# lgautier/fastq-and-furious

Hardware: AMD Instinct MI355X
Metric: GB/s FASTQ parsed (higher is better)
Workload: dtype u8; 1 GPU; single-1g; description=S-single 150 bp synthetic FASTQ, 1073741522 bytes/GPU, 3334601 records/GPU, diagnostic=False, bytes_per_gpu=1073741522, records_per_gpu=3334601, total_bytes=1073741522, total_records=3334601

## Files before the change

### fastq-and-furious_amd/csrc/ffq_hip.hip

```cpp
#include "../../include/ffq.h"
#ifdef FFQ_PROBES
#include "../../include/ffq_probe.h"
#endif
#include "ffq_kernels.h"
#include "ffq_fasta.h"
#include "ffq_pool.h"

#include <hip/hip_runtime.h>
#include <hip/hip_ext.h>
#include <sys/mman.h>
#include <sys/stat.h>
#include <unistd.h>
#include <algorithm>
#include <cctype>
#include <chrono>
#include <cstdarg>
#include <cstdio>
#include <cstring>
#include <cstdlib>
#include <new>
#include <string>
#include <vector>

using namespace ffq;
// ... 68 lines not shown
    bool dense4_remember = false;
    int fused_skip = 0;
    int fused_backoff = HOLD_OFF;
    bool fz_in_place = false;
};

struct ffq_ctx {
    ScanState pend;
    ffq_ctx *owner = nullptr;
    StreamTail tail;
    bool owns_streams = true;
    double watchdog_s = 0;
    int device = 0;
    hipStream_t stream = nullptr;
    hipEvent_t ev[7] = {nullptr, nullptr, nullptr, nullptr, nullptr, nullptr, nullptr};
    InputMemory mem;
    RankBufs rk = {};
    int64_t rk_cap_tiles = 0, rk_cap_c = 0;
    uint8_t *fz_qphase = nullptr;
    int64_t fz_tiles_cap = 0;
    uint32_t *fz_bad = nullptr;
    bool decode_timed = false;
    int64_t cap_tiles = 0;
    uint16_t *ent = nullptr;
    uint32_t *cnt = nullptr;
    unsigned long long *ovf = nullptr;
    uint16_t *pool = nullptr;
    unsigned long long pool_cap = 0;
    int64_t cap_groups = 0;
    ChainBufs cb = {};
    int64_t stage_cap = 0;
    int64_t dstage_chunks = 0;
    long long *sbbase = nullptr;
    TileQ *tileq = nullptr;
    unsigned int *sbq = nullptr;
    long long *sbqbase = nullptr;
    Fast4Hdr *hdr4 = nullptr;
    TermInfo4 *tinfo4 = nullptr;
    Ctl *ctl = nullptr;
    LineIndex *d_L = nullptr;
    LineIndex *h_L = nullptr;
    DevRes *dres = nullptr;
    int64_t *qdir = nullptr;
    int64_t qdir_cap = 0;
    int64_t *p4s = nullptr;
    int64_t p4s_cap = 0;
    uint32_t *qrel = nullptr;
    Ctl *h_ctl = nullptr;
    DevRes *h_res = nullptr;
    Ctl *hm_ctl = nullptr;
    DevRes *hm_res = nullptr;
    unsigned long long *h_seq = nullptr, *hm_seq = nullptr;
    unsigned long long seq = 0;
    unsigned long long pub_seq = 0;
    bool ctl_clean = false;
    bool ctl_was_clean = false;
    int64_t *d_word = nullptr;
    int64_t *h_word = nullptr;
    int64_t *d_cut = nullptr, *h_cut = nullptr;
    FaHdr *fa_hdr = nullptr;
    uint8_t *stage_d = nullptr;
    int64_t stage_d_cap = 0;
    uint8_t *stage_h = nullptr;
    int64_t stage_h_cap = 0;
    int64_t *tab_d = nullptr;
    int64_t tab_d_cap = 0;
// ... 72 lines not shown
    }
    for (int i = 0; i < 7 && e == hipSuccess; i++)
        e = (i == 2 || i == 3) ? hipEventCreate(&c->ev[i])
                               : hipEventCreateWithFlags(&c->ev[i], hipEventDisableSystemFence);
    if (e == hipSuccess) e = hipMalloc((void **)&c->ctl, sizeof(Ctl));
    if (e == hipSuccess) e = hipMalloc((void **)&c->dres, sizeof(DevRes));
    if (e == hipSuccess) e = hipMalloc((void **)&c->d_L, sizeof(LineIndex));
    if (e == hipSuccess) e = hipMalloc((void **)&c->d_word, 16);
    if (e == hipSuccess) e = hipHostMalloc((void **)&c->h_word, 16, hipHostMallocDefault);
    if (e == hipSuccess) e = hipMalloc((void **)&c->d_cut, 48);
    if (e == hipSuccess) e = hipMalloc((void **)&c->fa_hdr, sizeof(FaHdr));
    if (e == hipSuccess) e = hipHostMalloc((void **)&c->h_cut, 48, hipHostMallocDefault);
    if (e == hipSuccess) e = hipHostMalloc((void **)&c->h_L, sizeof(LineIndex), hipHostMallocDefault);
    if (e == hipSuccess) e = hipHostMalloc((void **)&c->h_ctl, sizeof(Ctl), hipHostMallocMapped);
    if (e == hipSuccess) e = hipHostMalloc((void **)&c->h_res, sizeof(DevRes), hipHostMallocMapped);
    if (e == hipSuccess) e = hipHostMalloc((void **)&c->h_seq, 64, hipHostMallocMapped);
    if (e == hipSuccess) { *c->h_seq = 0; e = hipHostGetDevicePointer((void **)&c->hm_seq, c->h_seq, 0); }
    if (e == hipSuccess) e = hipHostGetDevicePointer((void **)&c->hm_ctl, c->h_ctl, 0);
    if (e == hipSuccess) e = hipHostGetDevicePointer((void **)&c->hm_res, c->h_res, 0);
    if (e != hipSuccess) {
        ffq_ctx_destroy(c);
        return fail(FFQ_E_HIP, "context setup failed: %s", hipGetErrorString(e));
    }
    *out = c;
    return FFQ_OK;
}

static void free_chain(ffq_ctx *c)
{
    (void)hipFree(c->cb.y); (void)hipFree(c->cb.exit); (void)hipFree(c->cb.cnt); (void)hipFree(c->cb.flags);
    (void)hipFree(c->cb.lines); (void)hipFree(c->cb.qb); (void)hipFree(c->cb.term); (void)hipFree(c->cb.stage);
    (void)hipFree(c->cb.rloc); (void)hipFree(c->cb.qloc); (void)hipFree(c->cb.part); (void)hipFree(c->cb.mins);
    (void)hipFree(c->cb.force); (void)hipFree(c->cb.dlist); (void)hipFree(c->cb.ilist);
    (void)hipFree(c->sbbase); (void)hipFree(c->tinfo4);
    (void)hipFree(c->tileq); (void)hipFree(c->sbq); (void)hipFree(c->sbqbase);
    c->sbbase = nullptr; c->tinfo4 = nullptr;
    c->tileq = nullptr; c->sbq = nullptr; c->sbqbase = nullptr;
    {
        StageRec *ds = c->cb.dstage; const int32_t dc = c->cb.dchunks;
        c->cb = ChainBufs{};
        c->cb.dstage = ds; c->cb.dchunks = dc;
    }
    c->stage_cap = 0;
    c->cap_groups = 0;
}

extern "C" int ffq_ctx_create_shared(ffq_ctx *parent, ffq_ctx **out)
{
    if (!parent || !out) return fail(FFQ_E_ARG, "ffq_ctx_create_shared: NULL argument");
    return ctx_create_impl(parent->device, parent, out);
}

extern "C" void ffq_ctx_destroy(ffq_ctx *c)
{
    if (!c) return;
    (void)hipSetDevice(c->device);
    if (c->stream) (void)hipStreamSynchronize(c->stream);
    stream_cache_drop(c);
    for (auto &r : c->stage_ev) for (auto &e : r) if (e) (void)hipEventDestroy(e);
    for (auto &st : c->stage_cs) if (st) { (void)hipStreamSynchronize(st); (void)hipStreamDestroy(st); }
    delete c->helpers;
    (void)hipFree(c->ent); (void)hipFree(c->cnt); (void)hipFree(c->ovf); (void)hipFree(c->pool);
    (void)hipFree(c->rk.tbase); (void)hipFree(c->rk.cand); (void)hipFree(c->rk.rec); (void)hipFree(c->rk.succ);
    (void)hipFree(c->rk.S[0]); (void)hipFree(c->rk.S[1]); (void)hipFree(c->rk.C[0]); (void)hipFree(c->rk.C[1]);
    (void)hipFree(c->rk.D); (void)hipFree(c->rk.root);
    free_chain(c);
    (void)hipFree(c->cb.dstage);
    (void)hipFree(c->fz_qphase); (void)hipFree(c->fz_bad);
    (void)hipFree(c->ctl); (void)hipFree(c->dres); (void)hipFree(c->d_L); (void)hipFree(c->hdr4);
// ... 95 lines not shown
constexpr int NMAX_FAST = PER_FAST * 64, NMAX_DENSE = PER_DENSE * 64;
constexpr int WPB_LITE = 2;

static int reserve_tiles(ffq_ctx *c, int64_t ntiles)
{
    if (ntiles <= c->cap_tiles) return FFQ_OK;
    CTX_SYNC(c);
    (void)hipFree(c->ent); (void)hipFree(c->cnt); (void)hipFree(c->ovf);
    c->ent = nullptr; c->cnt = nullptr; c->ovf = nullptr;
    free_chain(c);
    c->cap_tiles = 0;
    const int64_t ng = groups_for(ntiles);
    const int64_t nblk = (ng + RES_BLOCK - 1) / RES_BLOCK;
    HIPCHK(hipMalloc((void **)&c->ent, (size_t)ntiles * SLOT * sizeof(uint16_t)));
    HIPCHK(hipMalloc((void **)&c->cnt, (size_t)ntiles * sizeof(uint32_t)));
    HIPCHK(hipMalloc((void **)&c->ovf, (size_t)ntiles * sizeof(unsigned long long)));
    HIPCHK(hipMalloc((void **)&c->cb.y, (size_t)ng * 8));
    HIPCHK(hipMalloc((void **)&c->cb.exit, (size_t)ng * 8));
    HIPCHK(hipMalloc((void **)&c->cb.cnt, (size_t)ng * 4));
    HIPCHK(hipMalloc((void **)&c->cb.flags, (size_t)(2 * ng + 8) * 4));
    HIPCHK(hipMalloc((void **)&c->cb.dlist, (size_t)ng * 4));
    HIPCHK(hipMalloc((void **)&c->cb.ilist, (size_t)ng * 4));
    HIPCHK(hipMalloc((void **)&c->cb.lines, (size_t)ng * 4));
    HIPCHK(hipMalloc((void **)&c->cb.qb, (size_t)ng * 8));
    HIPCHK(hipMalloc((void **)&c->cb.term, (size_t)ng * sizeof(GroupTerm)));
    HIPCHK(hipMalloc((void **)&c->cb.rloc, (size_t)ng * 8));
    HIPCHK(hipMalloc((void **)&c->cb.qloc, (size_t)ng * 8));
    HIPCHK(hipMalloc((void **)&c->cb.part, (size_t)nblk * 4 * 8));
    HIPCHK(hipMalloc((void **)&c->cb.mins, 16));
    HIPCHK(hipMalloc((void **)&c->cb.force, (size_t)ng * 8));
    {
        const int64_t nsb = (ntiles + SB_TILES - 1) / SB_TILES;
        HIPCHK(hipMalloc((void **)&c->sbbase, (size_t)nsb * sizeof(long long)));
        HIPCHK(hipMalloc((void **)&c->tinfo4, (size_t)ntiles * sizeof(TermInfo4)));
        HIPCHK(hipMalloc((void **)&c->tileq, (size_t)ntiles * sizeof(TileQ)));
        HIPCHK(hipMalloc((void **)&c->sbq, (size_t)nsb * sizeof(unsigned int)));
        HIPCHK(hipMalloc((void **)&c->sbqbase, (size_t)nsb * sizeof(long long)));
        if (!c->hdr4) HIPCHK(hipMalloc((void **)&c->hdr4, sizeof(Fast4Hdr)));
    }
    c->cap_tiles = ntiles;
    c->cap_groups = ng;
    return FFQ_OK;
}

static int reserve_dstage(ffq_ctx *c, int64_t chunks)
{
    if (chunks <= c->dstage_chunks) return FFQ_OK;
    CTX_SYNC(c);
    (void)hipFree(c->cb.dstage);
    c->cb.dstage = nullptr; c->dstage_chunks = 0; c->cb.dchunks = 0;
    hipError_t e = hipMalloc((void **)&c->cb.dstage, (size_t)chunks * DCHUNK * sizeof(StageRec));
    if (e != hipSuccess) return fail(FFQ_E_NOMEM, "hipMalloc(walked groups' stage, %lld chunks) failed: %s", (long long)chunks, hipGetErrorString(e));
    c->dstage_chunks = chunks;
    c->cb.dchunks = (int32_t)chunks;
    return FFQ_OK;
}

static int reserve_stage(ffq_ctx *c, int64_t ng, int nmax)
{
    const int64_t need = ng * nmax;
    if (need <= c->stage_cap) return FFQ_OK;
    CTX_SYNC(c);
    (void)hipFree(c->cb.stage);
    c->cb.stage = nullptr; c->stage_cap = 0;
    hipError_t e = hipMalloc((void **)&c->cb.stage, (size_t)need * sizeof(StageRec));
    if (e != hipSuccess) return fail(FFQ_E_NOMEM, "hipMalloc(stage) failed: %s", hipGetErrorString(e));
// ... 297 lines not shown
    int rc = reserve_stage(c, ngroups, nmax);
    if (rc) return rc;
    rc = reserve_dstage(c, 64);
    if (rc) return rc;
    ChainBufs cb = chain_bufs(c, ngroups, nmax);
    hipStream_t sA = c->stream;
    HIPCHK(hipMemsetAsync(cb.flags, 0, (2 * (size_t)ngroups + 3) * 4, sA));
    static const bool no_lite = getenv("FFQ_NO_LITE") != nullptr;
    bool lite = !dense_cfg && !no_lite;
    if (lite && c->mem.lite_skip > 0) { c->mem.lite_skip--; lite = false; }
    st.lite_ran = lite;
    if (lite) {
        const int gl = lite_first_end_group(a.n_bytes, L.ntiles, ngroups);
        hipLaunchKernelGGL(HIP_KERNEL_NAME(k_chain_lite<WPB_LITE>), dim3((ngroups + WPB_LITE - 1) / WPB_LITE), dim3(WPB_LITE * 64), 0, sA,
                           L, a.offset, cb, ngroups, gl);
    }
    if (lite)
        hipLaunchKernelGGL(HIP_KERNEL_NAME(k_chain_wave_list<PER_FAST, EMAX_FAST, WPB_FAST, false>),
                           dim3(std::min((ngroups + WPB_FAST - 1) / WPB_FAST, 4096)), dim3(WPB_FAST * 64), 0, sA, L,
                           (const LineIndex *)c->d_L, a.offset, a.eof, cb);
    else if (!dense_cfg)
        hipLaunchKernelGGL(HIP_KERNEL_NAME(k_chain_wave<PER_FAST, EMAX_FAST, WPB_FAST, false>),
                           dim3((ngroups + WPB_FAST - 1) / WPB_FAST), dim3(WPB_FAST * 64), 0, sA, L,
                           (const LineIndex *)c->d_L, a.offset, a.eof, cb, 0, ngroups, 0);
    else
        hipLaunchKernelGGL(HIP_KERNEL_NAME(k_chain_wave<PER_DENSE, EMAX_DENSE, WPB_DENSE, true>),
                           dim3((ngroups + WPB_DENSE - 1) / WPB_DENSE), dim3(WPB_DENSE * 64), 0, sA, L,
                           (const LineIndex *)c->d_L, a.offset, a.eof, cb, 0, ngroups, 0);
    hipLaunchKernelGGL(k_dense_walk, dim3((unsigned)std::min((ngroups + 3) / 4, 1024)), dim3(256), 0, sA, L, cb, a.offset, a.eof, 1,
                       dense_cfg ? 1 : 0, c->ctl, 1);
    return enqueue_resolve(c, st, cb, timed, lite);
}

static void enqueue_sbscan(ffq_ctx *c, const LineIndex &L, int64_t ntiles, int nsb, int64_t offset)
{
    const unsigned int *presum = nullptr;
    if (nsb > 2048) {
        hipLaunchKernelGGL(k_sum64, dim3((unsigned)((nsb + 3) / 4)), dim3(256), 0, c->stream, (const uint32_t *)c->cnt, 1,
                           (int64_t)ntiles, c->sbq, nsb);
        presum = c->sbq;
    }
    hipLaunchKernelGGL(k_sbscan, dim3(1), dim3(1024), 0, c->stream, L, nsb, c->sbbase, offset, c->hdr4, presum);
}

static int end_front(ffq_ctx *c, const ScanState &st)
{
    const ScanArgs &a = st.a;
    c->pub_seq = 0;
    if (!st.poll_seq) HIPCHK(hipEventRecord(c->ev[3], c->stream));
    HIPCHK(hipGetLastError());
    StreamTail &tl = c->owner->tail;
    tl.is_scan = true;
    tl.out_p[0] = a.d_table; tl.out_n[0] = (size_t)a.table_cap * 48;
    tl.out_p[1] = st.decode ? a.d_qual : nullptr; tl.out_n[1] = st.decode ? (size_t)a.qual_cap : 0;
    tl.out_p[2] = st.decode ? a.d_qoff : nullptr; tl.out_n[2] = st.decode ? ((size_t)a.table_cap + 1) * 8 : 0;
    return FFQ_OK;
}

static int enqueue_front(ffq_ctx *c, ScanState &st)
{
    const ScanArgs &a = st.a;
    const bool serial = st.serial, decode = st.decode;
    hipStream_t sA = c->stream;
    const int64_t ntiles = st.ntiles;
    const int nsb = (int)((ntiles + SB_TILES - 1) / SB_TILES);
    if (c->mem.ranked_skip > 0 && !serial && !st.index_done) { c->mem.ranked_skip--; st.go_ranked = true; }
    if (st.force_ranked && !serial) st.go_ranked = true;
    st.probe4 = false;
    if (c->mem.fast4_remember && !st.fast4_failed) {
        st.fast4_failed = true;
        if (c->mem.fast4_skip > 0) c->mem.fast4_skip--;
        else st.probe4 = !serial && !st.go_ranked && !st.index_done;
    }
    if (c->mem.dense_skip > 0 && !st.dense_cfg && !st.index_done) { c->mem.dense_skip--; st.dense_cfg = true; }
    const bool try_fast4 = !serial && !st.go_ranked && !st.dense_cfg && !st.fast4_failed && !st.force_general &&
                           getenv("FFQ_NO_FAST4") == nullptr;
    const LineIndex L = make_index(c, a, ntiles);
    c->decode_timed = false;
    st.poll_seq = (st.poll_result && !decode) ? ++c->seq : 0;
    c->pub_seq = st.poll_seq;
    c->ctl_was_clean = c->ctl_clean;
    if (!c->ctl_clean) HIPCHK(hipMemsetAsync(c->ctl, 0, sizeof(Ctl), sA));
    c->ctl_clean = false;

    st.fused = false;
    st.in_place = (c->mem.fz_in_place || st.seg_refused) && a.qual_cap >= ntiles * (int64_t)TILE;
    if (decode && st.single_pass && try_fast4 && !st.index_done && !st.no_fused && a.offset < 16 &&
        (st.in_place || (!st.seg_refused && a.qual_cap >= ntiles * (int64_t)SG_STRIDE)) && (reinterpret_cast<uintptr_t>(a.d_qual) & 15) == 0) {
        if (c->mem.fused_skip > 0) c->mem.fused_skip--;
        else st.fused = true;
    }
    if (st.fused) {
        int rc = enqueue_fused_index(c, a, ntiles, st.in_place);
        if (rc) return rc;
        enqueue_sbscan(c, L, ntiles, nsb, a.offset);
        auto rows4 = st.in_place ? k_rows4<2, false> : k_rows4<1, false>;
        hipLaunchKernelGGL(rows4, dim3((unsigned)((ntiles + 3) / 4)), dim3(256), 0, sA, L,
                           (const long long *)c->sbbase, a.eof, a.add, c->hdr4, c->tinfo4, a.d_table, a.table_cap,
                           (uint32_t *)nullptr, c->tileq, (int64_t *)nullptr, a.table_cap,
                           (int64_t)(st.in_place ? TILE : SG_STRIDE), (const uint8_t *)c->fz_qphase, a.d_qoff);
        hipLaunchKernelGGL(k_finalize4, dim3(1), dim3(64), 0, sA, L, c->hdr4, (const TermInfo4 *)c->tinfo4, a.eof,
                           a.offset, a.add, (const int64_t *)a.d_table, a.table_cap, c->dres, no_pub(c), (const uint32_t *)c->fz_bad);
        hipLaunchKernelGGL(k_qtotal4, dim3(1), dim3(1), 0, sA, c->dres, (const int64_t *)a.d_table, a.table_cap,
                           a.d_qoff, make_pub(c));
        c->ctl_clean = true;
        st.stage = 1;
        return end_front(c, st);
    }

    st.untimed = st.no_timing && st.poll_seq && !st.index_done;
    bool any_order = st.untimed && c->ctl_was_clean;
    {
        const StreamTail &tl = c->owner->tail;
        if (!tl.is_scan || tl.exposed) any_order = false;
        const uintptr_t b0 = reinterpret_cast<uintptr_t>(a.d_buf), b1 = b0 + (size_t)a.n_bytes;
        for (int i = 0; i < 3 && any_order; i++) {
            const uintptr_t o0 = reinterpret_cast<uintptr_t>(tl.out_p[i]), o1 = o0 + tl.out_n[i];
            if (tl.out_p[i] && o0 < b1 && b0 < o1) any_order = false;
        }
    }
    static const bool no_wide = getenv("FFQ_NO_WIDE") != nullptr;
    if (!st.index_done)
        st.wide = decode && st.single_pass && !try_fast4 && !no_wide &&
                  a.qual_cap >= ntiles * (int64_t)TILE && (reinterpret_cast<uintptr_t>(a.d_qual) & 15) == 0;
    if (!st.untimed) HIPCHK(hipEventRecord(c->ev[0], sA));
    if (!st.index_done)
        launch_scan_lines(c, sA, a.d_buf, a.n_bytes, ntiles, L, (uint32_t)'@', any_order && !st.wide,
                          st.wide ? a.d_qual : (int8_t *)nullptr, a.qual_add);
    if (!st.untimed) HIPCHK(hipEventRecord(c->ev[1], sA));

    if (try_fast4) {
        enqueue_sbscan(c, L, ntiles, nsb, a.offset);
        if (decode) HIPCHK(hipMemsetAsync(c->tileq, 0, (size_t)ntiles * sizeof(TileQ), sA));
        if (c->mem.dense4_remember) st.dense4 = true;
        auto rows4 = st.dense4 ? k_rows4<false, true> : k_rows4<false, false>;
        hipLaunchKernelGGL(rows4, dim3((unsigned)((ntiles + 3) / 4)), dim3(256), 0, sA, L,
                           (const long long *)c->sbbase, a.eof, a.add, c->hdr4, c->tinfo4, a.d_table, a.table_cap,
                           decode ? c->qrel : (uint32_t *)nullptr, c->tileq, decode ? c->p4s : (int64_t *)nullptr,
                           decode ? std::min<int64_t>(a.table_cap, c->p4s_cap) : (int64_t)0,
                           (int64_t)0, (const uint8_t *)nullptr, (int64_t *)nullptr);
        hipLaunchKernelGGL(k_finalize4, dim3(1), dim3(64), 0, sA, L, c->hdr4, (const TermInfo4 *)c->tinfo4, a.eof,
                           a.offset, a.add, (const int64_t *)a.d_table, a.table_cap, c->dres,
                           decode ? no_pub(c) : make_pub(c));
        if (decode) {
            hipLaunchKernelGGL(k_sum64, dim3((unsigned)((nsb + 3) / 4)), dim3(256), 0, sA,
                               reinterpret_cast<const uint32_t *>(c->tileq) + 3, 4, (int64_t)ntiles, c->sbq, nsb);
            hipLaunchKernelGGL(k_qscan4, dim3(1), dim3(1024), 0, sA, (const unsigned int *)c->sbq, nsb, c->sbqbase);
            hipLaunchKernelGGL(k_qfix4, dim3((unsigned)((ntiles + 7) / 8)), dim3(256), 0, sA, (int)ntiles,
                               (const Fast4Hdr *)c->hdr4, (const TileQ *)c->tileq, (const long long *)c->sbqbase,
                               (const uint32_t *)c->qrel, a.d_qoff, std::min<int64_t>(a.table_cap, c->p4s_cap), c->qdir,
                               c->qdir_cap);
            hipLaunchKernelGGL(k_qtotal4, dim3(1), dim3(1), 0, sA, c->dres, (const int64_t *)a.d_table, a.table_cap,
                               a.d_qoff, make_pub(c));
            enqueue_decode(c, a, sA, true);
        }
        c->ctl_clean = true;
        st.stage = 1;
    } else {
        if (st.probe4) {
            enqueue_sbscan(c, L, ntiles, nsb, a.offset);
            auto rows4 = c->mem.dense4_remember ? k_rows4<false, true> : k_rows4<false, false>;
            hipLaunchKernelGGL(rows4, dim3((unsigned)((ntiles + 3) / 4)), dim3(256), 0, sA, L,
                               (const long long *)c->sbbase, a.eof, a.add, c->hdr4, c->tinfo4, a.d_table, a.table_cap,
                               (uint32_t *)nullptr, c->tileq, (int64_t *)nullptr, (int64_t)0,
                               (int64_t)0, (const uint8_t *)nullptr, (int64_t *)nullptr);
            hipLaunchKernelGGL(k_finalize4, dim3(1), dim3(64), 0, sA, L, c->hdr4, (const TermInfo4 *)c->tinfo4, a.eof,
                               a.offset, a.add, (const int64_t *)a.d_table, a.table_cap, c->dres, no_pub(c));
        }
        if (!serial && !st.go_ranked) {
            int rc = enqueue_general(c, st, L, true);
            if (rc) return rc;
        } else {
            hipLaunchKernelGGL(k_publish, dim3(1), dim3(1), 0, sA, c->dres, make_pub(c), 1);
            c->ctl_clean = true;
        }
        st.stage = 2;
    }
    return end_front(c, st);
}

template <class T>
static int grow_dev(ffq_ctx *c, T **p, int64_t *cap, int64_t need);

static int launch_scan_i64v(ffq_ctx *c, hipStream_t st, long long *v, int64_t nv, int64_t n_rows, DevRes *res)
{
    if (nv <= 2 * 32768) {
        hipLaunchKernelGGL(k_scan_i64v, dim3(1), dim3(1024), 0, st, v, nv, n_rows, res);
        return FFQ_OK;
    }
    const int64_t nb = (nv + SCAN_BLK - 1) / SCAN_BLK;
    int rc = grow_dev(c, &c->scan_bs, &c->scan_bs_cap, nb);
    if (rc) return rc;
    hipLaunchKernelGGL(k_scan_blksum, dim3((unsigned)nb), dim3(256), 0, st, (const long long *)v, nv, c->scan_bs);
    hipLaunchKernelGGL(k_scan_i64v, dim3(1), dim3(1024), 0, st, c->scan_bs, nb, n_rows, res);
    hipLaunchKernelGGL(k_scan_blkapply, dim3((unsigned)nb), dim3(256), 0, st, v, nv, (const long long *)c->scan_bs);
    return FFQ_OK;
}

static int launch_scan_u32(ffq_ctx *c, hipStream_t st, const unsigned int *v, int64_t nv, long long *base, long long *total)
// ... 942 lines not shown
```

### fastq-and-furious_amd/csrc/ffq_rows4.h

```cpp
#pragma once
#include "ffq_chain.h"

namespace ffq {

constexpr int SB_TILES = 64;
constexpr int R4_LIST = SLOT + 8;

struct Fast4Hdr {
    long long j0;
    int32_t attempt;
    int32_t dense_seen;
    unsigned long long irr_min;
    unsigned long long term_min;
    long long n_lines;
};

struct TermInfo4 {
    int64_t pos[6];
    int32_t status;
    int32_t final_;
};

struct TileQ {
    long long kfirst;
    int32_t nrec;
    uint32_t qsum;
};

__device__ __forceinline__ long long tile_ordinal_base(const LineIndex &L, const long long *sbbase, int t, int lane)
{
    const int sb = t / SB_TILES, t0 = sb * SB_TILES;
    const uint32_t c = (t0 + lane < t) ? L.cnt[t0 + lane] : 0u;
    return sbbase[sb] + (long long)wave_sum_u32(c) + L.s;
}

__global__ __launch_bounds__(256) void k_sum64(const uint32_t *__restrict__ src, int stride, int64_t nsrc,
                                               unsigned int *__restrict__ dst, int ndst)
{
    const int b = blockIdx.x * 4 + __builtin_amdgcn_readfirstlane((int)(threadIdx.x >> 6)), lane = threadIdx.x & 63;
    if (b >= ndst) return;
    const int64_t i = (int64_t)b * 64 + lane;
    const uint32_t v = (i < nsrc) ? src[i * stride] : 0u;
    const uint32_t t = wave_sum_u32(v);
    if (lane == 0) dst[b] = t;
}

__global__ __launch_bounds__(1024) void k_sbscan(LineIndex L, int nsb, long long *__restrict__ sbbase, int64_t offset,
                                                 Fast4Hdr *hdr, const unsigned int *__restrict__ presum)
{
    __shared__ long long s_w[16];
    __shared__ uint32_t s_sum[16][64];
    const int tid = threadIdx.x, lane = tid & 63, wid = tid >> 6;
    if (wid == 15) {
        const int tq = (int)min((int64_t)max(L.ntiles - 1, 0), max((int64_t)0, (offset - L.s) >> TILE_SHIFT));
        uint32_t sink = (L.n > 0) ? (uint32_t)L.d[0] : 0u;
        if (L.ntiles > 0) sink += L.cnt[tq] + L.ent[(int64_t)tq * SLOT + lane * 4];
        if (tq + 1 < L.ntiles) sink += L.cnt[tq + 1] + L.ent[(int64_t)(tq + 1) * SLOT + (lane & 15) * 4];
        asm volatile("" ::"v"(sink));
    }
    long long carry = 0;
    if (presum) {
        for (int c0 = 0; c0 < nsb; c0 += 16 * 1024) {
            uint32_t pv[16];
#pragma unroll
            for (int k = 0; k < 16; k++) {
                const int b = c0 + k * 1024 + tid;
                pv[k] = (b < nsb) ? presum[b] : 0u;
            }
#pragma unroll
            for (int k = 0; k < 16; k++) {
                const int b = c0 + k * 1024 + tid;
                if (c0 + k * 1024 >= nsb) continue;
                const uint32_t v = pv[k];
                const uint32_t incl = wave_incl_scan(v);
                if (lane == 63) s_w[wid] = (long long)incl;
                __syncthreads();
                long long wpre = 0, tot = 0;
// ... 27 lines not shown
                for (int q = 0; q < 4; q++)
                    if (t + q < L.ntiles) a += L.cnt[t + q];
                part[j] = a;
            }
        }
#pragma unroll
        for (int j = 0; j < 16; j++) {
            uint32_t r = part[j];
            r += (uint32_t)__builtin_amdgcn_update_dpp(0, (int)r, 0x111, 0xf, 0xf, false);
            r += (uint32_t)__builtin_amdgcn_update_dpp(0, (int)r, 0x112, 0xf, 0xf, false);
            r += (uint32_t)__builtin_amdgcn_update_dpp(0, (int)r, 0x114, 0xf, 0xf, false);
            r += (uint32_t)__builtin_amdgcn_update_dpp(0, (int)r, 0x118, 0xf, 0xf, false);
            if ((lane & 15) == 15) s_sum[wid][4 * j + (lane >> 4)] = r;
        }
        __syncthreads();
        const uint32_t v = (b < nsb) ? s_sum[wid][lane] : 0u;
        const uint32_t incl = wave_incl_scan(v);
        if (lane == 63) s_w[wid] = (long long)incl;
        __syncthreads();
        long long wpre = 0, tot = 0;
#pragma unroll
        for (int q = 0; q < 16; q++) {
            const long long t = s_w[q];
            if (q < wid) wpre += t;
            tot += t;
        }
        if (b < nsb) sbbase[b] = carry + wpre + (long long)(incl - v);
        __syncthreads();
        carry += tot;
    }
    __syncthreads();
    if (tid == 0) {
        hdr->n_lines = carry;
        hdr->irr_min = ~0ull;
        hdr->term_min = ~0ull;
        hdr->attempt = 1;
        hdr->dense_seen = 0;
        hdr->j0 = -1;
        const GAcc a(L);
        H h = a.before();
        long long ord = -1;
        long long found = -1;
        int64_t P; int fl;
        int tskip = (int)min((int64_t)L.ntiles, max((int64_t)0, (offset - L.s) >> TILE_SHIFT));
        if (tskip > 0) {
            long long o = sbbase[tskip / SB_TILES] + L.s;
            for (int t = (tskip / SB_TILES) * SB_TILES; t < tskip; t++) o += L.cnt[t];
            h = H{tskip - 1, 0x7FFFFFF0};
            ord = o - 1;
        }
        bool gave_up = false;
        for (int steps = 0;; steps++) {
            if (steps > 4096) { gave_up = true; break; }
            bool ok;
            if (h.tile >= 0 && h.i == 0x7FFFFFF0) {
                int t = h.tile + 1;
                while (t < L.ntiles && L.cnt[t] == 0) t++;
                ok = t < L.ntiles;
                if (ok) { h.tile = t; h.i = 0; }
            } else ok = a.next(h);
            if (!ok) break;
            ord++;
            a.get(h, P, fl);
            if ((fl & FL_AT) && P >= offset) { found = ord; break; }
        }
        if (gave_up) hdr->attempt = 0;
        else {
            hdr->j0 = found;
            if (found >= 0) {
                H h2 = h;
                if (a.next(h2) && a.next(h2)) {
                    a.get(h2, P, fl);
                    if (!(fl & FL_PLUS)) hdr->attempt = 0;
                }
            }
        }
    }
}

constexpr uint8_t FZ_ALL = 0xFE;
template <int FUSED, bool DENSE>
__global__ __launch_bounds__(256, DENSE ? 4 : 8) void k_rows4(LineIndex L, const long long *__restrict__ sbbase, int eof,
                                               int64_t add, Fast4Hdr *hdr, TermInfo4 *__restrict__ tinfo,
                                               int64_t *__restrict__ table, int64_t table_cap,
                                               uint32_t *__restrict__ qrel, TileQ *__restrict__ tileq,
                                               int64_t *__restrict__ p4s, int64_t p4_cap,
                                               int64_t fz_stride, const uint8_t *__restrict__ fz_phase,
                                               int64_t *__restrict__ fz_qoff)
{
    __shared__ __attribute__((aligned(16))) uint16_t s_ent_all[4][R4_LIST];
    __shared__ uint32_t s_la_all[4][8];
    __shared__ __attribute__((aligned(16))) int32_t s_rows_all[4][64 * 6];
    const int wid = __builtin_amdgcn_readfirstlane((int)(threadIdx.x >> 6)), lane = threadIdx.x & 63;
    const int t = blockIdx.x * 4 + wid;
    if (t >= L.ntiles) return;
    const int attempt = hdr->attempt;
    const long long j0 = hdr->j0;
    const unsigned long long irr0 = hdr->irr_min;
    const unsigned long long term0 = hdr->term_min;
    uint16_t *s_ent = s_ent_all[wid];
    uint32_t *s_la = s_la_all[wid];
    int32_t *s_rows = s_rows_all[wid];
    const int64_t len = L.len();

    const int tn = min(t + 1, L.ntiles - 1);
    const int sb = t / SB_TILES, t0 = sb * SB_TILES;
    const uint16_t *src = L.ent + (int64_t)t * SLOT;
    const uint32_t c_raw = L.cnt[t];
    const uint2 v0 = *reinterpret_cast<const uint2 *>(src + 4 * lane);
    const uint32_t c1_raw = L.cnt[tn];
    const uint2 vla_raw = *reinterpret_cast<const uint2 *>(L.ent + (int64_t)tn * SLOT + 4 * (lane & 1));
    const uint32_t cb_raw = L.cnt[min(t0 + lane, L.ntiles - 1)];
    const long long sbb = sbbase[sb];
    constexpr bool fused = FUSED != 0, in_place = FUSED == 2;
    uint32_t fzph = 0;
    if (fused) fzph = fz_phase[t];
    asm volatile("" ::"v"(c_raw), "v"(v0.x), "v"(v0.y), "v"(c1_raw), "v"(vla_raw.x), "v"(vla_raw.y), "v"(cb_raw),
                 "v"(sbb), "s"(attempt), "s"(j0), "v"(fzph));
    const int c = (int)c_raw;
    const bool have_next = t + 1 < L.ntiles;
    const int c1 = have_next ? (int)c1_raw : 0;
    const uint2 vla = vla_raw;
    const long long ob = sbb + (long long)wave_sum_u32((t0 + lane < t) ? cb_raw : 0u) + L.s;
    if (!attempt) return;
    if (ob - j0 > 0 && ((unsigned long long)((ob - j0) >> 2) > irr0 || (unsigned long long)((ob - j0) >> 2) > (term0 >> 24))) return;
    if (c > SLOT && (!DENSE || fused)) {
        if (lane == 0 && (hdr->irr_min != 0ull || !hdr->dense_seen)) { atomicMin(&hdr->irr_min, 0ull); hdr->dense_seen = 1; }
        return;
    }
    if (fused) {
        const uint32_t want = (uint32_t)(((j0 + 3 - ob) % 4 + 4) % 4);
        const bool wrong = in_place ? (fzph != (uint32_t)FZ_ALL && fzph != want) : (c > 0 && fzph != want);
        if ((wrong || j0 != 0) && lane == 0 && hdr->irr_min != 0ull) atomicMin(&hdr->irr_min, 0ull);
    }
    const int pre = (t == 0 && L.s) ? 1 : 0;
    if (c + pre == 0 && t != 0) return;
    const int64_t tbase = ((int64_t)t << TILE_SHIFT) + L.s;
    const int64_t tb_add = tbase + add;
    const int32_t lim = (int32_t)min(len - tbase, (int64_t)0x7FFFFFF0);
    if (j0 < 0) {
        if (t == 0 && lane == 0) {
            TermInfo4 &ti = tinfo[0];
            for (int i = 0; i < 6; i++) ti.pos[i] = -1;
            ti.status = ST_HEAD_BEG; ti.final_ = 0;
            atomicMin(&hdr->term_min, 0ull);
        }
        return;
    }
    const int ntot = pre + c;
    const int nch = DENSE ? (ntot + SLOT - 1) / SLOT : 1;
    const uint16_t *dsrc = nullptr;
    if (DENSE && c > SLOT) {
        const unsigned long long at = L.ovf[t] & OVF_MASK;
        if (at + (unsigned long long)c > L.pool_cap) {
            if (lane == 0) atomicMin(&hdr->irr_min, 0ull);
            return;
// ... 336 lines not shown
        if (r + 1 >= me.nrec) nxt = me.qsum;
        else if (lane == 63) nxt = (idx + 1 < table_cap) ? (int64_t)qrel[idx + 1] : (int64_t)me.qsum;
        if (act) {
            qoff[idx] = base + loc;
            qdir_mark(qdir, qdir_cap, base + loc, nxt - loc, idx);
        }
    };
    auto rest = [&](const TileQ &me, int64_t base) {
        for (int r0 = 64; r0 < me.nrec; r0 += 64) {
            const int64_t idx = me.kfirst + r0 + lane;
            const bool act = r0 + lane < me.nrec && idx < table_cap;
            fix(me, base, r0, act ? (int64_t)qrel[idx] : 0, act);
        }
    };
    if (me0.nrec > 0) fix(me0, base0, 0, l0, a0);
    if (me1.nrec > 0) fix(me1, base1, 0, l1, a1);
    if (me0.nrec > 64) rest(me0, base0);
    if (me1.nrec > 64) rest(me1, base1);
}

__global__ void k_qtotal4(DevRes *res, const int64_t *__restrict__ table, int64_t table_cap,
                          int64_t *__restrict__ qoff, Pub pb)
{
    if (threadIdx.x != 0 || blockIdx.x != 0) return;
    if (res->fallback) { publish(pb, res); return; }
    const int64_t n = res->n_records;
    int64_t tot = 0;
    if (n > 0 && n <= table_cap) tot = qoff[n - 1] + (table[(n - 1) * 6 + 5] - table[(n - 1) * 6 + 4]);
    res->n_qual_bytes = tot;
    if (n <= table_cap) qoff[n] = tot;
    publish(pb, res);
}

__global__ void k_finalize4(LineIndex L, Fast4Hdr *hdr, const TermInfo4 *__restrict__ tinfo, int eof,
                            int64_t offset, int64_t add, const int64_t *__restrict__ table, int64_t table_cap,
                            DevRes *res, Pub pb, const uint32_t *__restrict__ fz_bad = nullptr)
{
    if (threadIdx.x != 0 || blockIdx.x != 0) return;
    res->n_lines = hdr->n_lines;
    res->n_qual_bytes = 0;
    res->term_group = -1;
    res->has_final = 0;
    const unsigned long long tm = hdr->term_min, im = hdr->irr_min;
    const unsigned long long tk = tm >> 24;
    res->fused_bad = fz_bad ? (int32_t)*fz_bad : 0;
    res->fast4_dense = hdr->dense_seen;
    if (!hdr->attempt || tm == ~0ull || (im != ~0ull && im <= tk) || (fz_bad && *fz_bad)) { res->fallback = 1; res->fast4_hint = 0; publish(pb, res); return; }
    res->fallback = 0;
    res->fast4_hint = 1;
    const int tt = (int)(tm & 0xFFFFFF);
    const TermInfo4 ti = tinfo[tt];
    const int status = ti.status;
    res->last_status = status;
    for (int i = 0; i < 6; i++) res->last_pos[i] = (ti.pos[i] >= 0) ? ti.pos[i] + add : -1;
    const long long ncomplete = (long long)tk;
    res->n_records = ncomplete + (ti.final_ ? 1 : 0);
    res->has_final = ti.final_ ? 1 : 0;
    int end;
    if (ti.final_) end = 0;
    else if (status == ST_HEAD_BEG) end = eof ? 0 : 1;
    else if (eof) end = (status == ST_QUAL_END) ? 2 : (status == ST_INVALID) ? 4 : 3;
    else end = (status == ST_INVALID) ? 4 : 1;
    res->end_state = end;
    if (ncomplete > 0 && ncomplete <= table_cap) res->end_offset = table[(ncomplete - 1) * 6 + 5] - add - 1;
    else res->end_offset = offset;
    publish(pb, res);
}

}
```

Measured before the change: 4976 GB/s.

## Replace single-block superblock scan with multi-block two-level ordinal base

```diff
diff --git a/fastq-and-furious_amd/csrc/ffq_hip.hip b/fastq-and-furious_amd/csrc/ffq_hip.hip
--- a/fastq-and-furious_amd/csrc/ffq_hip.hip
+++ b/fastq-and-furious_amd/csrc/ffq_hip.hip
@@ -124,6 +124,8 @@
     int64_t stage_cap = 0;
     int64_t dstage_chunks = 0;
     long long *sbbase = nullptr;
+    uint32_t *sbsum = nullptr;
+    uint32_t *blksum = nullptr;
     TileQ *tileq = nullptr;
     unsigned int *sbq = nullptr;
     long long *sbqbase = nullptr;
@@ -262,9 +264,9 @@
     (void)hipFree(c->cb.lines); (void)hipFree(c->cb.qb); (void)hipFree(c->cb.term); (void)hipFree(c->cb.stage);
     (void)hipFree(c->cb.rloc); (void)hipFree(c->cb.qloc); (void)hipFree(c->cb.part); (void)hipFree(c->cb.mins);
     (void)hipFree(c->cb.force); (void)hipFree(c->cb.dlist); (void)hipFree(c->cb.ilist);
-    (void)hipFree(c->sbbase); (void)hipFree(c->tinfo4);
+    (void)hipFree(c->sbbase); (void)hipFree(c->tinfo4); (void)hipFree(c->sbsum); (void)hipFree(c->blksum);
     (void)hipFree(c->tileq); (void)hipFree(c->sbq); (void)hipFree(c->sbqbase);
-    c->sbbase = nullptr; c->tinfo4 = nullptr;
+    c->sbbase = nullptr; c->tinfo4 = nullptr; c->sbsum = nullptr; c->blksum = nullptr;
     c->tileq = nullptr; c->sbq = nullptr; c->sbqbase = nullptr;
     {
         StageRec *ds = c->cb.dstage; const int32_t dc = c->cb.dchunks;
@@ -426,6 +428,8 @@
     {
         const int64_t nsb = (ntiles + SB_TILES - 1) / SB_TILES;
         HIPCHK(hipMalloc((void **)&c->sbbase, (size_t)nsb * sizeof(long long)));
+        HIPCHK(hipMalloc((void **)&c->sbsum, (size_t)nsb * sizeof(uint32_t)));
+        HIPCHK(hipMalloc((void **)&c->blksum, (size_t)OB_MAXBLK * sizeof(uint32_t)));
         HIPCHK(hipMalloc((void **)&c->tinfo4, (size_t)ntiles * sizeof(TermInfo4)));
         HIPCHK(hipMalloc((void **)&c->tileq, (size_t)ntiles * sizeof(TileQ)));
         HIPCHK(hipMalloc((void **)&c->sbq, (size_t)nsb * sizeof(unsigned int)));
@@ -789,8 +793,16 @@
     return enqueue_resolve(c, st, cb, timed, lite);
 }
 
-static void enqueue_sbscan(ffq_ctx *c, const LineIndex &L, int64_t ntiles, int nsb, int64_t offset)
-{
+static OrdBase enqueue_obase(ffq_ctx *c, const LineIndex &L, int64_t ntiles, int nsb, int64_t offset)
+{
+    OrdBase ob{c->sbbase, c->sbsum, c->blksum, 0};
+    const int64_t nblk = (ntiles + BLK_TILES - 1) / BLK_TILES;
+    if (nblk <= OB_MAXBLK && offset - L.s < TILE) {
+        hipLaunchKernelGGL(k_obase, dim3((unsigned)(nblk + 1)), dim3(64), 0, c->stream, L, (int)nblk, nsb, c->sbsum,
+                           c->blksum, offset, c->hdr4);
+        ob.nblk = (int32_t)nblk;
+        return ob;
+    }
     const unsigned int *presum = nullptr;
     if (nsb > 2048) {
         hipLaunchKernelGGL(k_sum64, dim3((unsigned)((nsb + 3) / 4)), dim3(256), 0, c->stream, (const uint32_t *)c->cnt, 1,
@@ -798,6 +810,7 @@
         presum = c->sbq;
     }
     hipLaunchKernelGGL(k_sbscan, dim3(1), dim3(1024), 0, c->stream, L, nsb, c->sbbase, offset, c->hdr4, presum);
+    return ob;
 }
 
 static int end_front(ffq_ctx *c, const ScanState &st)
@@ -850,13 +863,13 @@
     if (st.fused) {
         int rc = enqueue_fused_index(c, a, ntiles, st.in_place);
         if (rc) return rc;
-        enqueue_sbscan(c, L, ntiles, nsb, a.offset);
+        const OrdBase ob = enqueue_obase(c, L, ntiles, nsb, a.offset);
         auto rows4 = st.in_place ? k_rows4<2, false> : k_rows4<1, false>;
         hipLaunchKernelGGL(rows4, dim3((unsigned)((ntiles + 3) / 4)), dim3(256), 0, sA, L,
-                           (const long long *)c->sbbase, a.eof, a.add, c->hdr4, c->tinfo4, a.d_table, a.table_cap,
+                           ob, a.eof, a.add, c->hdr4, c->tinfo4, a.d_table, a.table_cap,
                            (uint32_t *)nullptr, c->tileq, (int64_t *)nullptr, a.table_cap,
                            (int64_t)(st.in_place ? TILE : SG_STRIDE), (const uint8_t *)c->fz_qphase, a.d_qoff);
-        hipLaunchKernelGGL(k_finalize4, dim3(1), dim3(64), 0, sA, L, c->hdr4, (const TermInfo4 *)c->tinfo4, a.eof,
+        hipLaunchKernelGGL(k_finalize4, dim3(1), dim3(64), 0, sA, L, c->hdr4, ob, (const TermInfo4 *)c->tinfo4, a.eof,
                            a.offset, a.add, (const int64_t *)a.d_table, a.table_cap, c->dres, no_pub(c), (const uint32_t *)c->fz_bad);
         hipLaunchKernelGGL(k_qtotal4, dim3(1), dim3(1), 0, sA, c->dres, (const int64_t *)a.d_table, a.table_cap,
                            a.d_qoff, make_pub(c));
@@ -887,16 +900,16 @@
     if (!st.untimed) HIPCHK(hipEventRecord(c->ev[1], sA));
 
     if (try_fast4) {
-        enqueue_sbscan(c, L, ntiles, nsb, a.offset);
+        const OrdBase ob = enqueue_obase(c, L, ntiles, nsb, a.offset);
         if (decode) HIPCHK(hipMemsetAsync(c->tileq, 0, (size_t)ntiles * sizeof(TileQ), sA));
         if (c->mem.dense4_remember) st.dense4 = true;
         auto rows4 = st.dense4 ? k_rows4<false, true> : k_rows4<false, false>;
         hipLaunchKernelGGL(rows4, dim3((unsigned)((ntiles + 3) / 4)), dim3(256), 0, sA, L,
-                           (const long long *)c->sbbase, a.eof, a.add, c->hdr4, c->tinfo4, a.d_table, a.table_cap,
+                           ob, a.eof, a.add, c->hdr4, c->tinfo4, a.d_table, a.table_cap,
                            decode ? c->qrel : (uint32_t *)nullptr, c->tileq, decode ? c->p4s : (int64_t *)nullptr,
                            decode ? std::min<int64_t>(a.table_cap, c->p4s_cap) : (int64_t)0,
                            (int64_t)0, (const uint8_t *)nullptr, (int64_t *)nullptr);
-        hipLaunchKernelGGL(k_finalize4, dim3(1), dim3(64), 0, sA, L, c->hdr4, (const TermInfo4 *)c->tinfo4, a.eof,
+        hipLaunchKernelGGL(k_finalize4, dim3(1), dim3(64), 0, sA, L, c->hdr4, ob, (const TermInfo4 *)c->tinfo4, a.eof,
                            a.offset, a.add, (const int64_t *)a.d_table, a.table_cap, c->dres,
                            decode ? no_pub(c) : make_pub(c));
         if (decode) {
@@ -915,13 +928,13 @@
         st.stage = 1;
     } else {
         if (st.probe4) {
-            enqueue_sbscan(c, L, ntiles, nsb, a.offset);
+            const OrdBase ob = enqueue_obase(c, L, ntiles, nsb, a.offset);
             auto rows4 = c->mem.dense4_remember ? k_rows4<false, true> : k_rows4<false, false>;
             hipLaunchKernelGGL(rows4, dim3((unsigned)((ntiles + 3) / 4)), dim3(256), 0, sA, L,
-                               (const long long *)c->sbbase, a.eof, a.add, c->hdr4, c->tinfo4, a.d_table, a.table_cap,
+                               ob, a.eof, a.add, c->hdr4, c->tinfo4, a.d_table, a.table_cap,
                                (uint32_t *)nullptr, c->tileq, (int64_t *)nullptr, (int64_t)0,
                                (int64_t)0, (const uint8_t *)nullptr, (int64_t *)nullptr);
-            hipLaunchKernelGGL(k_finalize4, dim3(1), dim3(64), 0, sA, L, c->hdr4, (const TermInfo4 *)c->tinfo4, a.eof,
+            hipLaunchKernelGGL(k_finalize4, dim3(1), dim3(64), 0, sA, L, c->hdr4, ob, (const TermInfo4 *)c->tinfo4, a.eof,
                                a.offset, a.add, (const int64_t *)a.d_table, a.table_cap, c->dres, no_pub(c));
         }
         if (!serial && !st.go_ranked) {
diff --git a/fastq-and-furious_amd/csrc/ffq_rows4.h b/fastq-and-furious_amd/csrc/ffq_rows4.h
--- a/fastq-and-furious_amd/csrc/ffq_rows4.h
+++ b/fastq-and-furious_amd/csrc/ffq_rows4.h
@@ -4,7 +4,16 @@
 namespace ffq {
 
 constexpr int SB_TILES = 64;
+constexpr int BLK_TILES = SB_TILES * 64;
+constexpr int OB_MAXBLK = 64;
 constexpr int R4_LIST = SLOT + 8;
+
+struct OrdBase {
+    const long long *sbbase;
+    const uint32_t *sbsum;
+    const uint32_t *blksum;
+    int32_t nblk;
+};
 
 struct Fast4Hdr {
     long long j0;
@@ -43,6 +52,53 @@
     const uint32_t v = (i < nsrc) ? src[i * stride] : 0u;
     const uint32_t t = wave_sum_u32(v);
     if (lane == 0) dst[b] = t;
+}
+
+__device__ void fast4_first(const LineIndex &L, const long long *sbbase, int64_t offset, Fast4Hdr *hdr)
+{
+    hdr->irr_min = ~0ull;
+    hdr->term_min = ~0ull;
+    hdr->attempt = 1;
+    hdr->dense_seen = 0;
+    hdr->j0 = -1;
+    const GAcc a(L);
+    H h = a.before();
+    long long ord = -1;
+    long long found = -1;
+    int64_t P; int fl;
+    int tskip = (int)min((int64_t)L.ntiles, max((int64_t)0, (offset - L.s) >> TILE_SHIFT));
+    if (tskip > 0) {
+        long long o = sbbase[tskip / SB_TILES] + L.s;
+        for (int t = (tskip / SB_TILES) * SB_TILES; t < tskip; t++) o += L.cnt[t];
+        h = H{tskip - 1, 0x7FFFFFF0};
+        ord = o - 1;
+    }
+    bool gave_up = false;
+    for (int steps = 0;; steps++) {
+        if (steps > 4096) { gave_up = true; break; }
+        bool ok;
+        if (h.tile >= 0 && h.i == 0x7FFFFFF0) {
+            int t = h.tile + 1;
+            while (t < L.ntiles && L.cnt[t] == 0) t++;
+            ok = t < L.ntiles;
+            if (ok) { h.tile = t; h.i = 0; }
+        } else ok = a.next(h);
+        if (!ok) break;
+        ord++;
+        a.get(h, P, fl);
+        if ((fl & FL_AT) && P >= offset) { found = ord; break; }
+    }
+    if (gave_up) hdr->attempt = 0;
+    else {
+        hdr->j0 = found;
+        if (found >= 0) {
+            H h2 = h;
+            if (a.next(h2) && a.next(h2)) {
+                a.get(h2, P, fl);
+                if (!(fl & FL_PLUS)) hdr->attempt = 0;
+            }
+        }
+    }
 }
 
 __global__ __launch_bounds__(1024) void k_sbscan(LineIndex L, int nsb, long long *__restrict__ sbbase, int64_t offset,
@@ -136,55 +192,86 @@
     __syncthreads();
     if (tid == 0) {
         hdr->n_lines = carry;
-        hdr->irr_min = ~0ull;
-        hdr->term_min = ~0ull;
-        hdr->attempt = 1;
-        hdr->dense_seen = 0;
-        hdr->j0 = -1;
-        const GAcc a(L);
-        H h = a.before();
-        long long ord = -1;
-        long long found = -1;
-        int64_t P; int fl;
-        int tskip = (int)min((int64_t)L.ntiles, max((int64_t)0, (offset - L.s) >> TILE_SHIFT));
-        if (tskip > 0) {
-            long long o = sbbase[tskip / SB_TILES] + L.s;
-            for (int t = (tskip / SB_TILES) * SB_TILES; t < tskip; t++) o += L.cnt[t];
-            h = H{tskip - 1, 0x7FFFFFF0};
-            ord = o - 1;
-        }
-        bool gave_up = false;
-        for (int steps = 0;; steps++) {
-            if (steps > 4096) { gave_up = true; break; }
-            bool ok;
-            if (h.tile >= 0 && h.i == 0x7FFFFFF0) {
-                int t = h.tile + 1;
-                while (t < L.ntiles && L.cnt[t] == 0) t++;
-                ok = t < L.ntiles;
-                if (ok) { h.tile = t; h.i = 0; }
-            } else ok = a.next(h);
-            if (!ok) break;
-            ord++;
-            a.get(h, P, fl);
-            if ((fl & FL_AT) && P >= offset) { found = ord; break; }
-        }
-        if (gave_up) hdr->attempt = 0;
-        else {
-            hdr->j0 = found;
-            if (found >= 0) {
-                H h2 = h;
-                if (a.next(h2) && a.next(h2)) {
-                    a.get(h2, P, fl);
-                    if (!(fl & FL_PLUS)) hdr->attempt = 0;
-                }
-            }
-        }
-    }
+        fast4_first(L, sbbase, offset, hdr);
+    }
+}
+
+__global__ __launch_bounds__(64) void k_obase(LineIndex L, int nblk, int nsb, uint32_t *__restrict__ sbsum,
+                                              uint32_t *__restrict__ blksum, int64_t offset, Fast4Hdr *hdr)
+{
+    const int lane = threadIdx.x;
+    if (blockIdx.x == 0) {
+        const bool have0 = L.ntiles > 0;
+        const uint32_t c0 = have0 ? L.cnt[0] : 0u;
+        const uint2 v = have0 ? *reinterpret_cast<const uint2 *>(L.ent + 4 * lane) : make_uint2(0u, 0u);
+        const uint8_t b0 = L.n > 0 ? L.d[0] : 0;
+        const int nin = (c0 <= (uint32_t)SLOT) ? min((int)c0, 256) : 0;
+        const uint32_t x[4] = {v.x & 0xFFFFu, v.x >> 16, v.y & 0xFFFFu, v.y >> 16};
+        int q0 = 4;
+#pragma unroll
+        for (int q = 3; q >= 0; q--)
+            if (4 * lane + q < nin && ((x[q] >> 14) & FL_AT) && (int64_t)(x[q] & OFF_MASK) + L.s >= offset) q0 = q;
+        const unsigned long long m = __ballot(q0 < 4);
+        long long j0 = -1;
+        int e2 = -1;
+        if (L.s && b0 == '@' && offset <= 0) { j0 = 0; e2 = 1; }
+        else if (m != 0ull) {
+            const int fl = __ffsll((long long)m) - 1;
+            const int i = 4 * fl + __shfl(q0, fl);
+            j0 = L.s + i; e2 = i + 2;
+        }
+        const bool decided = e2 >= 0 && e2 < nin;
+        const uint32_t w = (uint32_t)__shfl((int)((e2 & 2) ? v.y : v.x), (e2 >> 2) & 63);
+        const uint32_t fl2 = ((e2 & 1) ? (w >> 16) : (w & 0xFFFFu)) >> 14;
+        if (lane == 0) {
+            if (decided) {
+                hdr->irr_min = ~0ull;
+                hdr->term_min = ~0ull;
+                hdr->dense_seen = 0;
+                hdr->j0 = j0;
+                hdr->attempt = (fl2 & FL_PLUS) ? 1 : 0;
+            } else fast4_first(L, nullptr, offset, hdr);
+        }
+        return;
+    }
+    const int b = blockIdx.x - 1;
+    const int64_t tw0 = (int64_t)b * BLK_TILES + lane * 4;
+    uint32_t part[16];
+    if ((int64_t)(b + 1) * BLK_TILES <= L.ntiles) {
+        uint4 xx[16];
+#pragma unroll
+        for (int j = 0; j < 16; j++) xx[j] = *reinterpret_cast<const uint4 *>(L.cnt + tw0 + ((int64_t)j << 8));
+#pragma unroll
+        for (int j = 0; j < 16; j++) part[j] = xx[j].x + xx[j].y + xx[j].z + xx[j].w;
+    } else {
+#pragma unroll
+        for (int j = 0; j < 16; j++) {
+            const int64_t t = tw0 + ((int64_t)j << 8);
+            uint32_t a = 0;
+            for (int q = 0; q < 4; q++)
+                if (t + q < L.ntiles) a += L.cnt[t + q];
+            part[j] = a;
+        }
+    }
+    uint32_t tot = 0;
+#pragma unroll
+    for (int j = 0; j < 16; j++) {
+        uint32_t r = part[j];
+        tot += r;
+        r += (uint32_t)__builtin_amdgcn_update_dpp(0, (int)r, 0x111, 0xf, 0xf, false);
+        r += (uint32_t)__builtin_amdgcn_update_dpp(0, (int)r, 0x112, 0xf, 0xf, false);
+        r += (uint32_t)__builtin_amdgcn_update_dpp(0, (int)r, 0x114, 0xf, 0xf, false);
+        r += (uint32_t)__builtin_amdgcn_update_dpp(0, (int)r, 0x118, 0xf, 0xf, false);
+        const int s = b * 64 + 4 * j + (lane >> 4);
+        if ((lane & 15) == 15 && s < nsb) sbsum[s] = r;
+    }
+    tot = wave_sum_u32(tot);
+    if (lane == 0) blksum[b] = tot;
 }
 
 constexpr uint8_t FZ_ALL = 0xFE;
 template <int FUSED, bool DENSE>
-__global__ __launch_bounds__(256, DENSE ? 4 : 8) void k_rows4(LineIndex L, const long long *__restrict__ sbbase, int eof,
+__global__ __launch_bounds__(256, DENSE ? 4 : 8) void k_rows4(LineIndex L, const OrdBase obase, int eof,
                                                int64_t add, Fast4Hdr *hdr, TermInfo4 *__restrict__ tinfo,
                                                int64_t *__restrict__ table, int64_t table_cap,
                                                uint32_t *__restrict__ qrel, TileQ *__restrict__ tileq,
@@ -209,23 +296,30 @@
 
     const int tn = min(t + 1, L.ntiles - 1);
     const int sb = t / SB_TILES, t0 = sb * SB_TILES;
+    const int blk = t / BLK_TILES, s0 = blk * 64;
     const uint16_t *src = L.ent + (int64_t)t * SLOT;
     const uint32_t c_raw = L.cnt[t];
     const uint2 v0 = *reinterpret_cast<const uint2 *>(src + 4 * lane);
     const uint32_t c1_raw = L.cnt[tn];
     const uint2 vla_raw = *reinterpret_cast<const uint2 *>(L.ent + (int64_t)tn * SLOT + 4 * (lane & 1));
     const uint32_t cb_raw = L.cnt[min(t0 + lane, L.ntiles - 1)];
-    const long long sbb = sbbase[sb];
+    const uint32_t sbs_raw = obase.sbsum[min(s0 + lane, (L.ntiles - 1) / SB_TILES)];
+    const uint32_t bls_raw = obase.blksum[min(lane, OB_MAXBLK - 1)];
+    const long long sbb_raw = obase.sbbase[sb];
     constexpr bool fused = FUSED != 0, in_place = FUSED == 2;
     uint32_t fzph = 0;
     if (fused) fzph = fz_phase[t];
     asm volatile("" ::"v"(c_raw), "v"(v0.x), "v"(v0.y), "v"(c1_raw), "v"(vla_raw.x), "v"(vla_raw.y), "v"(cb_raw),
-                 "v"(sbb), "s"(attempt), "s"(j0), "v"(fzph));
+                 "v"(sbs_raw), "v"(bls_raw), "v"(sbb_raw), "s"(attempt), "s"(j0), "v"(fzph));
     const int c = (int)c_raw;
     const bool have_next = t + 1 < L.ntiles;
     const int c1 = have_next ? (int)c1_raw : 0;
     const uint2 vla = vla_raw;
-    const long long ob = sbb + (long long)wave_sum_u32((t0 + lane < t) ? cb_raw : 0u) + L.s;
+    const bool two = obase.nblk > 0;
+    const long long sbb = two ? 0ll : sbb_raw;
+    const uint32_t lsum = ((t0 + lane < t) ? cb_raw : 0u) + ((two && s0 + lane < sb) ? sbs_raw : 0u) +
+                          ((two && lane < blk) ? bls_raw : 0u);
+    const long long ob = sbb + (long long)wave_sum_u32(lsum) + L.s;
     if (!attempt) return;
     if (ob - j0 > 0 && ((unsigned long long)((ob - j0) >> 2) > irr0 || (unsigned long long)((ob - j0) >> 2) > (term0 >> 24))) return;
     if (c > SLOT && (!DENSE || fused)) {
@@ -628,12 +722,18 @@
     publish(pb, res);
 }
 
-__global__ void k_finalize4(LineIndex L, Fast4Hdr *hdr, const TermInfo4 *__restrict__ tinfo, int eof,
+__global__ void k_finalize4(LineIndex L, Fast4Hdr *hdr, const OrdBase obase, const TermInfo4 *__restrict__ tinfo, int eof,
                             int64_t offset, int64_t add, const int64_t *__restrict__ table, int64_t table_cap,
                             DevRes *res, Pub pb, const uint32_t *__restrict__ fz_bad = nullptr)
 {
-    if (threadIdx.x != 0 || blockIdx.x != 0) return;
-    res->n_lines = hdr->n_lines;
+    if (blockIdx.x != 0) return;
+    long long n_lines = 0;
+    if (obase.nblk > 0) {
+        const uint32_t v = ((int)threadIdx.x < obase.nblk) ? obase.blksum[threadIdx.x] : 0u;
+        n_lines = (long long)wave_sum_u32(v & 0xFFFFu) + ((long long)wave_sum_u32(v >> 16) << 16);
+    }
+    if (threadIdx.x != 0) return;
+    res->n_lines = (obase.nblk > 0) ? n_lines : hdr->n_lines;
     res->n_qual_bytes = 0;
     res->term_group = -1;
     res->has_final = 0;
```

Result: faster. 5056 GB/s (median of 6 runs) (+1.6%).
